# ov2slam/ov2slam

Hardware: AMD Instinct MI355X
Metric: frames/sec tracking + local-BA iters/sec, EuRoC MH_01 stereo 'accurate', 1 GPU vs CPU ref (higher is better)
Workload: dtype u8/int32 fixed point + f32 (LK), f64 (BA)

## Files before the change

### ov2slam_amd/csrc/clahe.hip

```cpp
#include "common.hpp"
#include "xcd_map.hpp"
#include <math.h>
#include <mutex>
#include <type_traits>

#pragma clang fp contract(off)

__device__ __forceinline__ int c_reflect101(int p, int len)
{
    if (len == 1) return 0;
    while (p < 0 || p >= len) p = p < 0 ? -p : 2 * len - 2 - p;
    return p;
}

struct ClaheParams {
    int w, h, stride, tiles_x, tiles_y, tw, th, clip;
    float lut_scale, inv_tw, inv_th;
    long long src_item_stride, dst_item_stride;
    int dst_stride;
    int border;
    int batch, gx_lut;
    int ysplit;
    int nstrips, nlut;
    long long l1_delta;
// ... 165 lines not shown
    __shared__ __attribute__((aligned(16))) uint32_t hist_all[4][CH_MULTI_DW];
    const int wave = __builtin_amdgcn_readfirstlane(threadIdx.x >> 6), lane = threadIdx.x & 63;
    const int ntiles = P.tiles_x * P.tiles_y;
    int b, bx;
    ov2_xcd_map(blockIdx.x, P.gx_lut, P.batch, &b, &bx);
    uint8_t *lb = lut + (long long)b * ntiles * 256 + 4 * lane;
    clahe_lut_tiles<SRC_ALIGNED>(P, src + (long long)b * P.src_item_stride, hist_all[wave], lane, bx * 4 + wave, ntiles, 4 * P.gx_lut,
                                 [&](int t, uint32_t packed) { *(uint32_t *)(lb + (long long)t * 256) = packed; }, CH_NCOPY);
}

#define CLAHE_MAX_CELLS 48
#define CA_UNROLL 6
typedef float c_f32x2 __attribute__((ext_vector_type(2)));

__device__ __forceinline__ float c_ub(uint32_t q, int k) { return (float)((q >> (8 * k)) & 0xFFu); }

template <bool SRC_ALIGNED>
__global__ __launch_bounds__(512) void k_clahe_apply(ClaheParams P, const uint8_t *__restrict__ src, const uint8_t *__restrict__ lut,
                                                     uint8_t *__restrict__ dst)
{
    extern __shared__ __align__(16) unsigned char clahe_smem[];
    const int ncx = P.tiles_x + 1;
    uint32_t *lut4 = (uint32_t *)clahe_smem;
    int cy, b;
    ov2_xcd_map(blockIdx.x, (P.tiles_y + 1) * P.ysplit, P.batch, &b, &cy);
    const int part = cy % P.ysplit;
    cy /= P.ysplit;
    const int tid = threadIdx.x, nthr = blockDim.x;
    const int ty1 = max(cy - 1, 0), ty2 = min(cy, P.tiles_y - 1);
    const uint8_t *L = lut + (long long)b * P.tiles_x * P.tiles_y * 256;
    for (int e = tid; e < ncx * 64; e += nthr) {
        const int cx = e >> 6, v4 = (e & 63) * 4;
        const int tx1 = max(cx - 1, 0), tx2 = min(cx, P.tiles_x - 1);
        const uint32_t a = *(const uint32_t *)(L + (ty1 * P.tiles_x + tx1) * 256 + v4), bb = *(const uint32_t *)(L + (ty1 * P.tiles_x + tx2) * 256 + v4);
        const uint32_t c = *(const uint32_t *)(L + (ty2 * P.tiles_x + tx1) * 256 + v4), d = *(const uint32_t *)(L + (ty2 * P.tiles_x + tx2) * 256 + v4);
        const uint32_t ab01 = __builtin_amdgcn_perm(bb, a, 0x05010400u), ab23 = __builtin_amdgcn_perm(bb, a, 0x07030602u);
        const uint32_t cd01 = __builtin_amdgcn_perm(d, c, 0x05010400u), cd23 = __builtin_amdgcn_perm(d, c, 0x07030602u);
        c_u32x4 o;
        o.x = __builtin_amdgcn_perm(cd01, ab01, 0x05040100u); o.y = __builtin_amdgcn_perm(cd01, ab01, 0x07060302u);
        o.z = __builtin_amdgcn_perm(cd23, ab23, 0x05040100u); o.w = __builtin_amdgcn_perm(cd23, ab23, 0x07060302u);
        *(c_u32x4 *)(lut4 + (cx << 8) + v4) = o;
    }
    __syncthreads();
    int y0 = max(0, (int)floorf(((float)cy - 0.5f) * (float)P.th) - 1), y1 = min(P.h, (int)ceilf(((float)cy + 0.5f) * (float)P.th) + 2);
    while (y0 < y1 && (int)floorf((float)y0 * P.inv_th - 0.5f) + 1 != cy) y0++;
    while (y1 > y0 && (int)floorf((float)(y1 - 1) * P.inv_th - 0.5f) + 1 != cy) y1--;
    if (P.ysplit > 1) {
        const int chunk = (y1 - y0 + P.ysplit - 1) / P.ysplit;
        y0 = min(y1, y0 + part * chunk);
        y1 = min(y1, y0 + chunk);
    }
    const uint8_t *simg = src + (long long)b * P.src_item_stride;
    uint8_t *dimg = dst + (long long)b * P.dst_item_stride;
    const bool dst_aligned = ((P.dst_stride | (int)(size_t)dimg) & 3) == 0;
    constexpr bool src_aligned = SRC_ALIGNED;
    const uint8_t *simg_end = simg + (long long)(P.h - 1) * P.stride + P.w;
    const int ndw = (P.w + 3) >> 2;
    for (int dwi = tid; dwi < ndw; dwi += nthr) {
        const int xb = 4 * dwi;
        float xa[4], xa1[4];
        const uint32_t *lutc[4];
#pragma unroll
        for (int k = 0; k < 4; k++) {
            const int x = min(xb + k, P.w - 1);
            const float txf = (float)x * P.inv_tw - 0.5f;
            const int fx = (int)floorf(txf);
            xa[k] = txf - (float)fx; xa1[k] = 1.0f - xa[k];
            lutc[k] = lut4 + ((fx + 1) << 8);
        }
        const c_f32x2 XA01 = {xa[0], xa[1]}, XA23 = {xa[2], xa[3]}, XB01 = {xa1[0], xa1[1]}, XB23 = {xa1[2], xa1[3]};
        const bool full = dst_aligned && xb + 3 < P.w;
        auto load_rows = [&](int yb, uint32_t (&inr)[CA_UNROLL]) {
#pragma unroll
            for (int u = 0; u < CA_UNROLL; u++) {
                const int y = min(yb + u, y1 - 1);
                const uint8_t *sp = simg + (long long)y * P.stride + xb;
                uint32_t in = 0;
                if (src_aligned) in = *(const uint32_t *)sp;
                else {
                    const uint32_t ph = (uint32_t)((size_t)sp & 3);
                    const uint8_t *ap = sp - ph;
                    if (xb + 3 < P.w && ap + 8 <= simg_end) {
                        const uint32_t lo = *(const uint32_t *)ap, hi = *(const uint32_t *)(ap + 4);
                        in = __builtin_amdgcn_alignbyte(hi, lo, ph);
                    } else for (int k = 0; k < 4; k++) if (xb + k < P.w) in |= (uint32_t)sp[k] << (8 * k);
                }
                inr[u] = in;
            }
        };
        uint32_t inr[CA_UNROLL], nxt[CA_UNROLL];
        if (y0 < y1) load_rows(y0, inr);
        for (int yb = y0; yb < y1; yb += CA_UNROLL) {
            load_rows(yb + CA_UNROLL, nxt);
#pragma unroll
            for (int u = 0; u < CA_UNROLL; u++) {
                const int y = yb + u;
                if (y >= y1) break;
                const float tyf = (float)y * P.inv_th - 0.5f;
                const float ya = tyf - (float)(cy - 1), ya1 = 1.0f - ya;
                const c_f32x2 YA = {ya, ya}, YB = {ya1, ya1};
                uint8_t *drow = dimg + y * P.dst_stride;
                const uint32_t in = inr[u];
                const uint32_t q0 = lutc[0][in & 0xFF], q1 = lutc[1][(in >> 8) & 0xFF], q2 = lutc[2][(in >> 16) & 0xFF], q3 = lutc[3][in >> 24];
                const c_f32x2 A11 = {c_ub(q0, 0), c_ub(q1, 0)}, A12 = {c_ub(q0, 1), c_ub(q1, 1)}, A21 = {c_ub(q0, 2), c_ub(q1, 2)}, A22 = {c_ub(q0, 3), c_ub(q1, 3)};
                const c_f32x2 B11 = {c_ub(q2, 0), c_ub(q3, 0)}, B12 = {c_ub(q2, 1), c_ub(q3, 1)}, B21 = {c_ub(q2, 2), c_ub(q3, 2)}, B22 = {c_ub(q2, 3), c_ub(q3, 3)};
                const c_f32x2 r01 = (A11 * XB01 + A12 * XA01) * YB + (A21 * XB01 + A22 * XA01) * YA;
                const c_f32x2 r23 = (B11 * XB23 + B12 * XA23) * YB + (B21 * XB23 + B22 * XA23) * YA;
                uint32_t out = __builtin_amdgcn_cvt_pk_u8_f32(rintf(r01.x), 0, 0u);
                out = __builtin_amdgcn_cvt_pk_u8_f32(rintf(r01.y), 1, out);
                out = __builtin_amdgcn_cvt_pk_u8_f32(rintf(r23.x), 2, out);
                out = __builtin_amdgcn_cvt_pk_u8_f32(rintf(r23.y), 3, out);
                if (full) *(uint32_t *)(drow + xb) = out;
                else for (int k = 0; k < 4; k++) if (xb + k < P.w) drow[xb + k] = (uint8_t)(out >> (8 * k));
            }
#pragma unroll
            for (int u = 0; u < CA_UNROLL; u++) inr[u] = nxt[u];
        }
    }
    if (P.border > 0) {
        __threadfence_block();
        __syncthreads();
        const int win = P.border, pbl = (win + 3) & ~3, wend = (P.w + win + 3) & ~3, rbeg = P.w & ~3;
        const int ndw_lr = pbl / 4 + ((wend - rbeg) >> 2), ndw_row = (pbl + wend) >> 2;
        auto put = [&](int yt, int ysrc, int c0) {
            const uint8_t *srow = dimg + ysrc * P.dst_stride;
            uint32_t v;
            if (c0 >= 0 && c0 + 3 < P.w) v = *(const uint32_t *)(srow + c0);
            else {
                v = 0;
#pragma unroll
                for (int k = 0; k < 4; k++) {
                    int c = c0 + k;
                    c = c < -win ? -win : (c > P.w + win - 1 ? P.w + win - 1 : c);
                    v |= (uint32_t)srow[c_reflect101(c, P.w)] << (8 * k);
                }
            }
            *(uint32_t *)(dimg + yt * P.dst_stride + c0) = v;
        };
        for (int row = tid >> 3; row < y1 - y0; row += nthr >> 3)
            for (int d = tid & 7; d < ndw_lr; d += 8)
                put(y0 + row, y0 + row, d < pbl / 4 ? 4 * d - pbl : rbeg + 4 * (d - pbl / 4));
        for (int k = max(1, y0); k <= min(win, y1 - 1); k++)
            for (int d = tid; d < ndw_row; d += nthr) put(-k, k, 4 * d - pbl);
        for (int k = max(1, P.h - y1); k <= min(win, P.h - 1 - y0); k++)
            for (int d = tid; d < ndw_row; d += nthr) put(P.h - 1 + k, P.h - 1 - k, 4 * d - pbl);
    }
}

__device__ __forceinline__ uint32_t c_wave_shr1(uint32_t v) { return (uint32_t)__builtin_amdgcn_update_dpp(0, (int)v, 0x138, 0xF, 0xF, true); }
__device__ __forceinline__ uint32_t c_wave_shl1(uint32_t v) { return (uint32_t)__builtin_amdgcn_update_dpp(0, (int)v, 0x130, 0xF, 0xF, true); }

#define CS_UNROLL 6
#define CS_MAX_STRIPS 8
#define CS_LUT_PRIO 3
template <bool UNAL, bool FUSED>
__global__ __launch_bounds__(64 * (CS_MAX_STRIPS + 2), 6) void k_clahe_apply_pyr(ClaheParams P, const uint8_t *__restrict__ src, const uint8_t *__restrict__ lut,
                                                                                uint8_t *__restrict__ dst)
{
    extern __shared__ __align__(16) unsigned char clahe_smem[];
    uint32_t *lut4 = (uint32_t *)clahe_smem;
    uint8_t *ring = clahe_smem + (size_t)(P.tiles_x + 1) * 1024;
    const int b = blockIdx.x, s = __builtin_amdgcn_readfirstlane(threadIdx.x >> 6);
    const int lane = threadIdx.x & 63, ndw = (P.w + 3) >> 2, wr = UNAL ? (P.w & 3) : 0;
    uint32_t *hist_w = (uint32_t *)(ring + (size_t)2 * P.tiles_x * 256) + (s < P.nstrips ? s * CH_WAVE_DW : P.nstrips * CH_WAVE_DW + (s - P.nstrips) * CH_MULTI_DW);
    const int hist_copies = s < P.nstrips ? 1 : CH_NCOPY;
    auto lut_row = [&](int ty, int tx0, int txstep) {
        uint8_t *slot = ring + (size_t)(ty & 1) * P.tiles_x * 256 - (size_t)ty * P.tiles_x * 256 + 4 * lane;
        clahe_lut_tiles<!UNAL>(P, src + (long long)b * P.src_item_stride, hist_w, lane, ty * P.tiles_x + tx0, (ty + 1) * P.tiles_x, txstep,
                               [&](int t, uint32_t packed) { *(uint32_t *)(slot + (size_t)t * 256) = packed; }, hist_copies);
    };
    typedef uint32_t cs_u32_a1 __attribute__((aligned(1)));
    const int cmin = 0, ncell = P.tiles_x + 1;
    const uint8_t *L = lut + (long long)b * P.tiles_x * P.tiles_y * 256;
    auto cell_row = [&](int y) { return (int)floorf((float)y * P.inv_th - 0.5f) + 1; };
    int cy = -1, y_switch = 0;
    auto build = [&](int cyv) {
        const int ty1 = max(cyv - 1, 0), ty2 = min(cyv, P.tiles_y - 1);
        const uint8_t *L1 = FUSED ? ring + (size_t)(ty1 & 1) * P.tiles_x * 256 : L + (size_t)ty1 * P.tiles_x * 256;
        const uint8_t *L2 = FUSED ? ring + (size_t)(ty2 & 1) * P.tiles_x * 256 : L + (size_t)ty2 * P.tiles_x * 256;
        __syncthreads();
        for (int e = threadIdx.x; e < ncell * 64; e += blockDim.x) {
            const int cx = cmin + (e >> 6), v4 = (e & 63) * 4;
            const int tx1 = max(cx - 1, 0), tx2 = min(cx, P.tiles_x - 1);
            const uint32_t a = *(const uint32_t *)(L1 + tx1 * 256 + v4), bb = *(const uint32_t *)(L1 + tx2 * 256 + v4);
            const uint32_t c = *(const uint32_t *)(L2 + tx1 * 256 + v4), dd = *(const uint32_t *)(L2 + tx2 * 256 + v4);
            const uint32_t ab01 = __builtin_amdgcn_perm(bb, a, 0x05010400u), ab23 = __builtin_amdgcn_perm(bb, a, 0x07030602u);
            const uint32_t cd01 = __builtin_amdgcn_perm(dd, c, 0x05010400u), cd23 = __builtin_amdgcn_perm(dd, c, 0x07030602u);
            c_u32x4 o;
            o.x = __builtin_amdgcn_perm(cd01, ab01, 0x05040100u); o.y = __builtin_amdgcn_perm(cd01, ab01, 0x07060302u);
            o.z = __builtin_amdgcn_perm(cd23, ab23, 0x05040100u); o.w = __builtin_amdgcn_perm(cd23, ab23, 0x07060302u);
            *(c_u32x4 *)(lut4 + ((e >> 6) << 8) + v4) = o;
        }
        __syncthreads();
    };
    if (FUSED) {
        lut_row(0, s, P.nstrips + P.nlut);
        if (s >= P.nstrips) {
            const int n_cell_rows = cell_row(P.h - 1) + 1;
            __builtin_amdgcn_s_setprio(CS_LUT_PRIO);
            for (int c = 0; c < n_cell_rows; c++) {
                build(c);
                if (c + 1 < P.tiles_y) lut_row(c + 1, s - P.nstrips, P.nlut);
            }
            return;
        }
    }
    const int core0 = s == 0 ? 0 : 63 + 62 * (s - 1);
    const int core1 = s == P.nstrips - 1 ? ndw : 63 + 62 * s;
    const int d_first = s == 0 ? 0 : core0 - 1;
    const int d_raw = d_first + lane;
    const int d = min(d_raw, ndw - 1);
    const bool core = d_raw >= core0 && d_raw < core1;
    const int xb = 4 * d;
    float xa[4], xa1[4];
    const uint32_t *lutc[4];
#pragma unroll
    for (int k = 0; k < 4; k++) {
        const float txf = (float)min(xb + k, P.w - 1) * P.inv_tw - 0.5f;
        const int fx = (int)floorf(txf);
        xa[k] = txf - (float)fx; xa1[k] = 1.0f - xa[k];
        lutc[k] = lut4 + ((fx + 1 - cmin) << 8);
    }
    const c_f32x2 XA01 = {xa[0], xa[1]}, XA23 = {xa[2], xa[3]}, XB01 = {xa1[0], xa1[1]}, XB23 = {xa1[2], xa1[3]};
    uint8_t *dimg = dst + (long long)b * P.dst_item_stride;
    uint8_t *l1 = dimg + P.l1_delta;
    const int win = P.border;
    const int l1odd = UNAL ? (P.l1_w & 1) : 0;
    const int nb0 = (win + 3) >> 2, nb1 = (win + 1) >> 1;
    const int nbr0 = nb0 + (wr ? 1 : 0), nbr1 = nb1 + l1odd;
    const bool bl0 = core && d < nb0, br0 = core && d >= ndw - nbr0;
    const bool bl1 = core && d >= 1 && d <= nb1, br1 = core && d >= ndw - nbr1;
    const bool edge_strip = s == 0 || core1 > ndw - max(nbr0, nbr1);
    const bool first_col = d_raw == 0, last_col = d_raw == ndw - 1;
    const bool dup = d_raw > ndw - 1;
    const uint32_t pad0 = 4u * nb0, pad1 = 2u * nb1;
    const uint32_t slack0 = pad0 + 4u * (uint32_t)((P.w + win + 3) >> 2), slack1 = pad1 + 2u * (uint32_t)((P.l1_w + win + 3) >> 1);
    const uint32_t o0 = dup ? slack0 : pad0 + 4u * d;
    const uint32_t o0b = bl0 ? pad0 - 4u * (d + 1) : (br0 ? pad0 + (uint32_t)(2 * P.w - 2 - xb - ((wr & 1) ? 0 : 2)) : slack0);
    const uint32_t sel_br = (wr & 1) ? 0x01020304u : 0x03040506u;
    const uint32_t sel_fix = (last_col && wr) ? (wr == 1 ? 0x01020304u : (wr == 2 ? 0x03040504u : 0x05060504u)) : 0x07060504u;
    const uint32_t sel_rt = wr == 0 ? 0x0c0c0c06u : (wr == 1 ? 0x0c0c0c00u : (wr == 2 ? 0x0c0c0c02u : 0x0c0c0c04u));
    const uint32_t o1 = core ? pad1 + 2u * d : slack1;
    const uint32_t o1b = bl1 ? pad1 - 2u * d : (br1 ? pad1 + (uint32_t)P.l1_w + 2u * (ndw - 1 - d) - (uint32_t)l1odd : slack1);
    const bool fix1 = last_col && l1odd;
    uint8_t *d0m = dimg - pad0, *d1m = l1 - pad1;
    const uint32_t xo = (d == ndw - 1 && wr) ? (uint32_t)(P.w - 4) : (uint32_t)xb;
    const uint32_t in_sh = (d == ndw - 1 && wr) ? 8u * (4u - (uint32_t)wr) : 0u;

    auto stage = [&](int y) {
        cy = cell_row(y);
        int yn = max(y + 1, (int)(((float)cy + 0.5f) * (float)P.th) - 2);
        while (yn < P.h && cell_row(yn) == cy) yn++;
        y_switch = yn;
        build(cy);
    };
    uint8_t *dbase = min(d0m - (long long)win * P.dst_stride, d1m - (long long)win * P.l1_pitch) - 256;
    const __amdgpu_buffer_rsrc_t rs_dst = __builtin_amdgcn_make_buffer_rsrc(dbase, 0, 0x7fffffff, 0x00020000);
    const uint8_t *sbase = src + (long long)b * P.src_item_stride;
    const __amdgpu_buffer_rsrc_t rs_src = __builtin_amdgcn_make_buffer_rsrc((void *)sbase, 0, 0x7fffffff, 0x00020000);
    auto put0 = [&](uint8_t *row, uint32_t v, uint32_t bv) {
        const int so = (int)(row - dbase);
        __builtin_amdgcn_raw_buffer_store_b32(v, rs_dst, (int)o0, so, 0);
        if (edge_strip) __builtin_amdgcn_raw_buffer_store_b32(bv, rs_dst, (int)o0b, so, 0);
    };
    auto put1 = [&](uint8_t *row, uint32_t v, uint32_t bv) {
        const int so = (int)(row - dbase);
        __builtin_amdgcn_raw_buffer_store_b16((unsigned short)v, rs_dst, (int)o1, so, 0);
        if (edge_strip) __builtin_amdgcn_raw_buffer_store_b16((unsigned short)bv, rs_dst, (int)o1b, so, 0);
    };
    typedef unsigned short cu16x2 __attribute__((ext_vector_type(2)));
    uint8_t *r1 = d1m;
    auto emit = [&](int Y, uint32_t c0, uint32_t c1, uint32_t c2, uint32_t c3, uint32_t c4, auto mirror_c) {
        constexpr bool MIRROR = decltype(mirror_c)::value;
        const cu16x2 s0 = __builtin_bit_cast(cu16x2, c0), s1 = __builtin_bit_cast(cu16x2, c1), s2 = __builtin_bit_cast(cu16x2, c2),
                     s3 = __builtin_bit_cast(cu16x2, c3), s4 = __builtin_bit_cast(cu16x2, c4);
        const cu16x2 v = (s2 * (unsigned short)6 + (s1 + s3) * (unsigned short)4 + s0 + s4 + (unsigned short)128) >> (unsigned short)8;
        uint32_t o = __builtin_amdgcn_perm(0u, __builtin_bit_cast(uint32_t, v), 0x0c0c0200u);
        uint32_t bv = 0;
        if (edge_strip) {
            bv = __builtin_amdgcn_perm(c_wave_shr1(o), o, 0x0c0c0500u);
            if (UNAL && fix1) o = bv;
        }
        put1(r1, o, bv);
        r1 += P.l1_pitch;
        if (MIRROR) {
            if (Y >= 1 && Y <= win) put1(d1m - (long long)Y * P.l1_pitch, o, bv);
            if (Y >= P.l1_h - 1 - win && Y <= P.l1_h - 2) put1(d1m + (long long)(2 * (P.l1_h - 1) - Y) * P.l1_pitch, o, bv);
        }
    };

    uint32_t hA = 0, hB = 0, hC = 0, hD = 0, hE = 0;
    const uint8_t *srow = src + (long long)b * P.src_item_stride;
    uint8_t *r0 = d0m;
    uint32_t inr[CS_UNROLL], nxt[CS_UNROLL];
#pragma unroll
    for (int u = 0; u < CS_UNROLL; u++) inr[u] = *(const cs_u32_a1 *)(srow + (long long)min(u, P.h - 1) * P.stride + xo) >> (UNAL ? in_sh : 0u);
    srow += (long long)CS_UNROLL * P.stride;
    auto do_row = [&](int y, uint32_t in, auto mirror_c) {
        constexpr bool MIRROR = decltype(mirror_c)::value;
        const float tyf = (float)y * P.inv_th - 0.5f;
        const float ya = tyf - (float)(cy - 1), ya1 = 1.0f - ya;
        const c_f32x2 YA = {ya, ya}, YB = {ya1, ya1};
        const uint32_t q0 = lutc[0][in & 0xFF], q1 = lutc[1][(in >> 8) & 0xFF], q2 = lutc[2][(in >> 16) & 0xFF], q3 = lutc[3][in >> 24];
        const c_f32x2 A11 = {c_ub(q0, 0), c_ub(q1, 0)}, A12 = {c_ub(q0, 1), c_ub(q1, 1)}, A21 = {c_ub(q0, 2), c_ub(q1, 2)}, A22 = {c_ub(q0, 3), c_ub(q1, 3)};
        const c_f32x2 B11 = {c_ub(q2, 0), c_ub(q3, 0)}, B12 = {c_ub(q2, 1), c_ub(q3, 1)}, B21 = {c_ub(q2, 2), c_ub(q3, 2)}, B22 = {c_ub(q2, 3), c_ub(q3, 3)};
        const c_f32x2 r01 = (A11 * XB01 + A12 * XA01) * YB + (A21 * XB01 + A22 * XA01) * YA;
        const c_f32x2 r23 = (B11 * XB23 + B12 * XA23) * YB + (B21 * XB23 + B22 * XA23) * YA;
        const c_f32x2 MAGIC = {12582912.0f, 12582912.0f};
        const c_f32x2 m01 = r01 + MAGIC, m23 = r23 + MAGIC;
        const uint32_t u0 = __builtin_bit_cast(uint32_t, (float)m01.x), u1 = __builtin_bit_cast(uint32_t, (float)m01.y);
        const uint32_t u2 = __builtin_bit_cast(uint32_t, (float)m23.x), u3 = __builtin_bit_cast(uint32_t, (float)m23.y);
        uint32_t out = __builtin_amdgcn_perm(__builtin_amdgcn_perm(u3, u2, 0x0c0c0400u), __builtin_amdgcn_perm(u1, u0, 0x0c0c0400u), 0x05040100u);
        uint32_t lf = c_wave_shr1(out), rt = c_wave_shl1(out);
        if (first_col) lf = __builtin_amdgcn_perm(out, out, 0x01020000u);
        if (edge_strip) {
            if (UNAL) out = __builtin_amdgcn_perm(out, lf, sel_fix);
        }
        if (UNAL) { if (last_col) rt = __builtin_amdgcn_perm(out, lf, sel_rt); }
        else if (last_col) rt = out >> 16;
        uint32_t bv = 0;
        if (edge_strip)
            bv = bl0 ? __builtin_amdgcn_perm(out, rt, 0x05060700u) : __builtin_amdgcn_perm(out, lf, sel_br);
        put0(r0, out, bv);
        r0 += P.dst_stride;
        if (MIRROR) {
            if (y >= 1 && y <= win) put0(d0m - (long long)y * P.dst_stride, out, bv);
            if (y >= P.h - 1 - win && y <= P.h - 2) put0(d0m + (long long)(2 * (P.h - 1) - y) * P.dst_stride, out, bv);
        }
        const uint32_t l0 = __builtin_amdgcn_alignbyte(out, lf, 2);
        const uint32_t h0 = __builtin_amdgcn_udot4(l0, 0x04060401u, __builtin_amdgcn_udot4(out, 0x00010000u, 0u, false), false);
        const uint32_t h1 = __builtin_amdgcn_udot4(out, 0x04060401u, __builtin_amdgcn_udot4(rt, 0x00000001u, 0u, false), false);
        hA = hB; hB = hC; hC = hD; hD = hE; hE = h0 | (h1 << 16);
    };
    for (int yb = 0; yb < P.h; yb += CS_UNROLL) {
        if (yb + 2 * CS_UNROLL <= P.h) {
#pragma unroll
            for (int u = 0; u < CS_UNROLL; u++) { nxt[u] = (uint32_t)__builtin_amdgcn_raw_buffer_load_b32(rs_src, (int)xo, (int)(srow - sbase), 0) >> (UNAL ? in_sh : 0u); srow += P.stride; }
        } else {
#pragma unroll
            for (int u = 0; u < CS_UNROLL; u++)
                nxt[u] = *(const cs_u32_a1 *)(src + (long long)b * P.src_item_stride + (long long)min(yb + CS_UNROLL + u, P.h - 1) * P.stride + xo) >> (UNAL ? in_sh : 0u);
        }
        if (yb == y_switch) stage(yb);
        const bool fast = yb > 2 * win + 2 && yb + CS_UNROLL - 1 < P.h - 1 - win && yb + CS_UNROLL - 4 < 2 * (P.l1_h - 1 - win) &&
                          y_switch >= yb + CS_UNROLL && yb + CS_UNROLL <= P.h;
        if (fast) {
#pragma unroll
            for (int u = 0; u < CS_UNROLL; u++) {
                do_row(yb + u, inr[u], std::false_type());
                if ((u & 1) == 0) emit((yb + u - 2) >> 1, hA, hB, hC, hD, hE, std::false_type());
            }
        } else {
#pragma nounroll
            for (int u = 0; u < CS_UNROLL; u++) {
                const int y = yb + u;
                if (y >= P.h) break;
                if (y == y_switch) stage(y);
                do_row(y, inr[0], std::true_type());
                if (!(y & 1)) {
                    if (y == 2) emit(0, hE, hD, hC, hD, hE, std::true_type());
                    else if (y > 2) emit((y - 2) >> 1, hA, hB, hC, hD, hE, std::true_type());
                }
#pragma unroll
                for (int k = 0; k + 1 < CS_UNROLL; k++) inr[k] = inr[k + 1];
            }
        }
#pragma unroll
        for (int u = 0; u < CS_UNROLL; u++) inr[u] = nxt[u];
    }
    if (P.h & 1) emit((P.h - 1) >> 1, hC, hD, hE, hD, hC, std::true_type());
    else emit((P.h - 2) >> 1, hB, hC, hD, hE, hD, std::true_type());
}

int ov2_launch_clahe(ov2_ctx *ctx, const uint8_t *src_d, int w, int h, int stride, size_t src_batch_stride, int batch,
                     double clip_limit, int tiles_x, int tiles_y, uint8_t *dst_d, int dst_stride, size_t dst_batch_stride,
                     uint8_t *lut_d, int border, const PyrDesc *pyr, int *level1_done)
{
    if (level1_done) *level1_done = 0;
    OV2_REQUIRE(tiles_x + 1 <= CLAHE_MAX_CELLS && (size_t)(tiles_x + 1) * 1024 <= 160 * 1024, OV2_EUNSUPPORTED,
                "CLAHE: too many tile columns / too wide an image for the LDS tables");
    static std::once_flag attr_once;
    static hipError_t attr_err = hipSuccess;
    std::call_once(attr_once, [] {
        attr_err = hipFuncSetAttribute((const void *)k_clahe_apply<true>, hipFuncAttributeMaxDynamicSharedMemorySize, 160 * 1024);
        if (attr_err == hipSuccess)
            attr_err = hipFuncSetAttribute((const void *)k_clahe_apply<false>, hipFuncAttributeMaxDynamicSharedMemorySize, 160 * 1024);
    });
    OV2_HIP_CHECK(attr_err);
    ClaheParams P;
    P.border = border;
    P.nstrips = 0; P.nlut = 0; P.l1_delta = 0; P.l1_pitch = P.l1_w = P.l1_h = 0;
    int ew = w, eh = h;
    if (!(w % tiles_x == 0 && h % tiles_y == 0)) { ew = w + (tiles_x - w % tiles_x); eh = h + (tiles_y - h % tiles_y); }
    P.w = w; P.h = h; P.stride = stride; P.tiles_x = tiles_x; P.tiles_y = tiles_y;
    P.tw = ew / tiles_x; P.th = eh / tiles_y;
    const int total = P.tw * P.th;
    P.lut_scale = (float)(256 - 1) / (float)total;
    P.clip = 0;
    if (clip_limit > 0.0) { P.clip = (int)(clip_limit * total / 256); if (P.clip < 1) P.clip = 1; }
    P.inv_tw = 1.0f / (float)P.tw; P.inv_th = 1.0f / (float)P.th;
    P.src_item_stride = (long long)src_batch_stride; P.dst_item_stride = (long long)dst_batch_stride; P.dst_stride = dst_stride;
    const int tiles_per_wave = (long long)batch * tiles_x * tiles_y >= 32768 ? 5 : 1;
    const bool src_al = ((stride | (int)(size_t)src_d | (int)src_batch_stride) & 3) == 0;
    P.ysplit = (long long)batch * (tiles_y + 1) >= 256 ? 1 : (P.th >= 48 ? 6 : (P.th >= 16 ? 3 : 1));
    P.batch = batch; P.gx_lut = (tiles_x * tiles_y + 4 * tiles_per_wave - 1) / (4 * tiles_per_wave);
    bool lut_launched = false;
    auto launch_lut = [&] {
        if (!lut_launched) hipLaunchKernelGGL(src_al ? k_clahe_lut<true> : k_clahe_lut<false>, dim3(P.gx_lut * batch), dim3(256), 0, ctx->stream, P, src_d, lut_d);
        lut_launched = true;
    };
    if (pyr && pyr->n_levels >= 2 && border == pyr->win && w >= 64 && h >= 8 && 2 * ((border + 3) / 4) + 1 <= (w + 3) / 4 &&
        (((size_t)dst_d | (size_t)dst_stride | dst_batch_stride) & 3) == 0 && (pyr->lv[1].img_pitch & 1) == 0) {
        const int ndw = (w + 3) / 4, nstrips = ndw <= 64 ? 1 : 2 + (ndw - 126 + 61) / 62;
        const bool want = ctx->clahe_strips >= 0 ? ctx->clahe_strips >= 1 : (long long)batch * nstrips >= 1024;
        if (want && nstrips <= CS_MAX_STRIPS && tiles_x + 1 <= 40) {
            static std::once_flag strip_once;
            static hipError_t strip_err = hipSuccess;
            std::call_once(strip_once, [] {
                const void *fn[4] = {(const void *)k_clahe_apply_pyr<false, false>, (const void *)k_clahe_apply_pyr<true, false>,
                                     (const void *)k_clahe_apply_pyr<false, true>, (const void *)k_clahe_apply_pyr<true, true>};
                for (int i = 0; i < 4 && strip_err == hipSuccess; i++) strip_err = hipFuncSetAttribute(fn[i], hipFuncAttributeMaxDynamicSharedMemorySize, 72 * 1024);
            });
            OV2_HIP_CHECK(strip_err);
            P.nstrips = nstrips;
            P.l1_delta = pyr->lv[1].img_roi - pyr->lv[0].img_roi; P.l1_pitch = pyr->lv[1].img_pitch; P.l1_w = pyr->lv[1].w; P.l1_h = pyr->lv[1].h;
            const bool unal = (w & 3) != 0 || (pyr->lv[1].w & 1) != 0;
            const int nlut = tiles_x <= 16 ? 1 : std::max(1, std::min((tiles_x + 7) / 8, CS_MAX_STRIPS + 2 - nstrips));
            const bool fused = (ctx->clahe_strips == 2 || (ctx->clahe_strips < 0 && tiles_x <= 16 * nlut)) && (unal || src_al);
            if (fused) {
                P.nlut = nlut;
                const size_t lds = (size_t)(tiles_x + 1) * 1024 + (size_t)2 * tiles_x * 256 + ((size_t)nstrips * CH_WAVE_DW + (size_t)P.nlut * CH_MULTI_DW) * 4;
                hipLaunchKernelGGL((unal ? k_clahe_apply_pyr<true, true> : k_clahe_apply_pyr<false, true>), dim3(batch), dim3(64 * (nstrips + P.nlut)), lds, ctx->stream, P, src_d, lut_d, dst_d);
            } else {
                launch_lut();
                hipLaunchKernelGGL((unal ? k_clahe_apply_pyr<true, false> : k_clahe_apply_pyr<false, false>), dim3(batch), dim3(64 * nstrips), (size_t)(tiles_x + 1) * 1024, ctx->stream, P, src_d, lut_d, dst_d);
            }
            OV2_HIP_CHECK(hipGetLastError());
            if (level1_done) *level1_done = 1;
            return OV2_OK;
        }
    }
    launch_lut();
    const size_t apply_lds = (size_t)(tiles_x + 1) * 1024;
    const int ndw = (w + 3) / 4, passes = (ndw + 511) / 512;
    const int apply_threads = (((ndw + passes - 1) / passes) + 63) / 64 * 64;
    hipLaunchKernelGGL(src_al ? k_clahe_apply<true> : k_clahe_apply<false>, dim3((tiles_y + 1) * P.ysplit * batch), dim3(apply_threads), apply_lds, ctx->stream, P, src_d, lut_d, dst_d);
    OV2_HIP_CHECK(hipGetLastError());
    return OV2_OK;
}

extern "C" {

int ov2_clahe_d(ov2_ctx *ctx, const uint8_t *src_d, int w, int h, int stride, size_t src_batch_stride, int batch,
                double clip_limit, int tiles_x, int tiles_y, uint8_t *dst_d, int dst_stride, size_t dst_batch_stride)
{
    OV2_REQUIRE(ctx && src_d && dst_d, OV2_EINVAL, "NULL argument");
    OV2_REQUIRE(w > 0 && h > 0 && stride >= w && dst_stride >= w && batch >= 1 && tiles_x > 0 && tiles_y > 0, OV2_EINVAL, "bad geometry");
    OV2_REQUIRE(tiles_x <= w && tiles_y <= h, OV2_EINVAL, "more tiles than pixels");
    OV2_HIP_CHECK(hipSetDevice(ctx->device));
    const size_t lut_bytes = (size_t)batch * tiles_x * tiles_y * 256;
    const int rc = ctx->reserve_device(lut_bytes);
    if (rc != OV2_OK) return rc;
    return ov2_launch_clahe(ctx, src_d, w, h, stride, src_batch_stride, batch, clip_limit, tiles_x, tiles_y, dst_d, dst_stride,
                            dst_batch_stride, (uint8_t *)ctx->d_scratch, 0, nullptr, nullptr);
}

int ov2_pyr_build_clahe_d(ov2_ctx *ctx, ov2_pyr *p, const uint8_t *img_d, int stride, size_t img_batch_stride,
                          double clip_limit, int tiles_x, int tiles_y)
{
    OV2_REQUIRE(ctx && p && img_d, OV2_EINVAL, "NULL argument");
    OV2_REQUIRE(stride >= p->w && tiles_x > 0 && tiles_y > 0 && tiles_x <= p->w && tiles_y <= p->h, OV2_EINVAL, "bad geometry");
    OV2_REQUIRE(p->d.batch == 1 || img_batch_stride >= (size_t)stride * (size_t)p->h, OV2_EINVAL, "img_batch_stride too small");
    OV2_HIP_CHECK(hipSetDevice(ctx->device));
    const size_t lut_bytes = (size_t)p->d.batch * tiles_x * tiles_y * 256;
    int rc = ctx->reserve_device(lut_bytes);
    if (rc != OV2_OK) return rc;
    const PyrLevelDesc &L0 = p->d.lv[0];
    int l1_done = 0;
    rc = ov2_launch_clahe(ctx, img_d, p->w, p->h, stride, img_batch_stride, p->d.batch, clip_limit, tiles_x, tiles_y,
                          p->d.base + L0.img_roi, L0.img_pitch, (size_t)p->d.item_stride, (uint8_t *)ctx->d_scratch, p->d.win,
                          &p->d, &l1_done);
    if (rc != OV2_OK) return rc;
    rc = ov2_launch_pyr_build(ctx, p, nullptr, 0, 0, l1_done);
    if (rc != OV2_OK) return rc;
    return ov2_pyr_mark_ready(ctx, p);
}

int ov2_pyr_build_clahe_h(ov2_ctx *ctx, ov2_pyr *p, const uint8_t *img_h, int stride, double clip_limit, int tiles_x, int tiles_y)
{
    OV2_REQUIRE(ctx && p && img_h, OV2_EINVAL, "NULL argument");
    OV2_REQUIRE(p->d.batch == 1, OV2_EINVAL, "host-buffer entry point takes batch=1 pyramids");
    OV2_REQUIRE(stride >= p->w && tiles_x > 0 && tiles_y > 0 && tiles_x <= p->w && tiles_y <= p->h, OV2_EINVAL, "bad geometry");
    OV2_HIP_CHECK(hipSetDevice(ctx->device));
    const size_t pitch = ((size_t)p->w + 15) & ~(size_t)15;
    const size_t img = (pitch * p->h + 255) & ~(size_t)255, lut_bytes = (size_t)tiles_x * tiles_y * 256;
    int rc = ctx->reserve_device(img + lut_bytes);
    if (rc != OV2_OK) return rc;
    uint8_t *ds = (uint8_t *)ctx->d_scratch;
    rc = ctx->upload_image(ds, pitch, img_h, (size_t)stride, (size_t)p->w, (size_t)p->h);
    if (rc != OV2_OK) return rc;
    const PyrLevelDesc &L0 = p->d.lv[0];
    int l1_done = 0;
    rc = ov2_launch_clahe(ctx, ds, p->w, p->h, (int)pitch, 0, 1, clip_limit, tiles_x, tiles_y, p->d.base + L0.img_roi, L0.img_pitch,
                          (size_t)p->d.item_stride, ds + img, p->d.win, &p->d, &l1_done);
    if (rc != OV2_OK) return rc;
    rc = ov2_launch_pyr_build(ctx, p, nullptr, 0, 0, l1_done);
    if (rc != OV2_OK) return rc;
    return ov2_pyr_mark_ready(ctx, p);
}

int ov2_pyr_build_clahe_hb(ov2_ctx *ctx, ov2_pyr *p, int n_items, const uint8_t *const *img_h, int stride, double clip_limit, int tiles_x, int tiles_y)
{
    OV2_REQUIRE(ctx && p && img_h, OV2_EINVAL, "NULL argument");
    OV2_REQUIRE(p->parent == nullptr, OV2_EINVAL, "an item view is read-only");
    OV2_REQUIRE(n_items >= 1 && n_items <= p->d.batch, OV2_EINVAL, "n_items out of range");
    const bool use_clahe = clip_limit >= 0.0;
    OV2_REQUIRE(stride >= p->w && (!use_clahe || (tiles_x > 0 && tiles_y > 0 && tiles_x <= p->w && tiles_y <= p->h)), OV2_EINVAL, "bad geometry");
    for (int b = 0; b < n_items; b++) OV2_REQUIRE(img_h[b] != nullptr, OV2_EINVAL, "NULL image");
    OV2_HIP_CHECK(hipSetDevice(ctx->device));
    const size_t pitch = ((size_t)p->w + 15) & ~(size_t)15;
    const size_t img = (pitch * p->h + 255) & ~(size_t)255, lut_bytes = use_clahe ? (size_t)n_items * tiles_x * tiles_y * 256 : 0;
    int rc = ctx->reserve_device(img * (size_t)n_items + lut_bytes);
    if (rc != OV2_OK) return rc;
    uint8_t *ds = (uint8_t *)ctx->d_scratch;
// ... 40 lines not shown
```

Measured before the change: 1.190 million.

## Specialize CLAHE apply loop on edge strips and prefetch LUT gathers ahead

Wraps the row walk of the fused CLAHE+pyramid kernel in a template lambda specialized on whether the wave handles an edge strip, so interior strips drop the per-row edge branches and extra stores. The LDS LUT gathers are split from the blend math and issued several rows ahead (all rows when fused, three otherwise) to hide LDS latency. All source loads now go through buffer loads, offsets are kept as 32-bit ints, and the fused variant's occupancy hint drops from 6 to 5 to allow more registers. The cost is larger code and higher register pressure, which may reduce occupancy.

```diff
diff --git a/ov2slam_amd/csrc/clahe.hip b/ov2slam_amd/csrc/clahe.hip
--- a/ov2slam_amd/csrc/clahe.hip
+++ b/ov2slam_amd/csrc/clahe.hip
@@ -341,9 +341,10 @@
 
 #define CS_UNROLL 6
 #define CS_MAX_STRIPS 8
+#define CS_AHEAD_PLAIN 3
 #define CS_LUT_PRIO 3
 template <bool UNAL, bool FUSED>
-__global__ __launch_bounds__(64 * (CS_MAX_STRIPS + 2), 6) void k_clahe_apply_pyr(ClaheParams P, const uint8_t *__restrict__ src, const uint8_t *__restrict__ lut,
+__global__ __launch_bounds__(64 * (CS_MAX_STRIPS + 2), FUSED ? 5 : 6) void k_clahe_apply_pyr(ClaheParams P, const uint8_t *__restrict__ src, const uint8_t *__restrict__ lut,
                                                                                 uint8_t *__restrict__ dst)
 {
     extern __shared__ __align__(16) unsigned char clahe_smem[];
@@ -358,7 +359,6 @@
         clahe_lut_tiles<!UNAL>(P, src + (long long)b * P.src_item_stride, hist_w, lane, ty * P.tiles_x + tx0, (ty + 1) * P.tiles_x, txstep,
                                [&](int t, uint32_t packed) { *(uint32_t *)(slot + (size_t)t * 256) = packed; }, hist_copies);
     };
-    typedef uint32_t cs_u32_a1 __attribute__((aligned(1)));
     const int cmin = 0, ncell = P.tiles_x + 1;
     const uint8_t *L = lut + (long long)b * P.tiles_x * P.tiles_y * 256;
     auto cell_row = [&](int y) { return (int)floorf((float)y * P.inv_th - 0.5f) + 1; };
@@ -428,6 +428,8 @@
     const uint32_t o0b = bl0 ? pad0 - 4u * (d + 1) : (br0 ? pad0 + (uint32_t)(2 * P.w - 2 - xb - ((wr & 1) ? 0 : 2)) : slack0);
     const uint32_t sel_br = (wr & 1) ? 0x01020304u : 0x03040506u;
     const uint32_t sel_fix = (last_col && wr) ? (wr == 1 ? 0x01020304u : (wr == 2 ? 0x03040504u : 0x05060504u)) : 0x07060504u;
+    const uint32_t sel_lf = first_col ? 0x05060404u : 0x03020100u;
+    const uint32_t sel_rt0 = last_col ? 0x0c0c0706u : 0x03020100u;
     const uint32_t sel_rt = wr == 0 ? 0x0c0c0c06u : (wr == 1 ? 0x0c0c0c00u : (wr == 2 ? 0x0c0c0c02u : 0x0c0c0c04u));
     const uint32_t o1 = core ? pad1 + 2u * d : slack1;
     const uint32_t o1b = bl1 ? pad1 - 2u * d : (br1 ? pad1 + (uint32_t)P.l1_w + 2u * (ndw - 1 - d) - (uint32_t)l1odd : slack1);
@@ -447,118 +449,127 @@
     const __amdgpu_buffer_rsrc_t rs_dst = __builtin_amdgcn_make_buffer_rsrc(dbase, 0, 0x7fffffff, 0x00020000);
     const uint8_t *sbase = src + (long long)b * P.src_item_stride;
     const __amdgpu_buffer_rsrc_t rs_src = __builtin_amdgcn_make_buffer_rsrc((void *)sbase, 0, 0x7fffffff, 0x00020000);
-    auto put0 = [&](uint8_t *row, uint32_t v, uint32_t bv) {
-        const int so = (int)(row - dbase);
-        __builtin_amdgcn_raw_buffer_store_b32(v, rs_dst, (int)o0, so, 0);
-        if (edge_strip) __builtin_amdgcn_raw_buffer_store_b32(bv, rs_dst, (int)o0b, so, 0);
+    const int d0o = (int)(d0m - dbase), d1o = (int)(d1m - dbase);
+    auto load_row = [&](int so) { return (uint32_t)__builtin_amdgcn_raw_buffer_load_b32(rs_src, (int)xo, so, 0) >> (UNAL ? in_sh : 0u); };
+    typedef unsigned short cu16x2 __attribute__((ext_vector_type(2)));
+
+    auto walk = [&](auto edge_c) {
+        constexpr bool EDGE = decltype(edge_c)::value;
+        auto put0 = [&](int so, uint32_t v, uint32_t bv) {
+            __builtin_amdgcn_raw_buffer_store_b32(v, rs_dst, (int)o0, so, 0);
+            if (EDGE) __builtin_amdgcn_raw_buffer_store_b32(bv, rs_dst, (int)o0b, so, 0);
+        };
+        auto put1 = [&](int so, uint32_t v, uint32_t bv) {
+            __builtin_amdgcn_raw_buffer_store_b16((unsigned short)v, rs_dst, (int)o1, so, 0);
+            if (EDGE) __builtin_amdgcn_raw_buffer_store_b16((unsigned short)bv, rs_dst, (int)o1b, so, 0);
+        };
+        int r1 = d1o;
+        auto emit = [&](int Y, uint32_t c0, uint32_t c1, uint32_t c2, uint32_t c3, uint32_t c4, auto mirror_c) {
+            constexpr bool MIRROR = decltype(mirror_c)::value;
+            const cu16x2 s0 = __builtin_bit_cast(cu16x2, c0), s1 = __builtin_bit_cast(cu16x2, c1), s2 = __builtin_bit_cast(cu16x2, c2),
+                         s3 = __builtin_bit_cast(cu16x2, c3), s4 = __builtin_bit_cast(cu16x2, c4);
+            const cu16x2 v = (s2 * (unsigned short)6 + (s1 + s3) * (unsigned short)4 + s0 + s4 + (unsigned short)128) >> (unsigned short)8;
+            uint32_t o = __builtin_amdgcn_perm(0u, __builtin_bit_cast(uint32_t, v), 0x0c0c0200u);
+            uint32_t bv = 0;
+            if (EDGE) {
+                bv = __builtin_amdgcn_perm(c_wave_shr1(o), o, 0x0c0c0500u);
+                if (UNAL && fix1) o = bv;
+            }
+            put1(r1, o, bv);
+            r1 += P.l1_pitch;
+            if (MIRROR) {
+                if (Y >= 1 && Y <= win) put1(d1o - Y * P.l1_pitch, o, bv);
+                if (Y >= P.l1_h - 1 - win && Y <= P.l1_h - 2) put1(d1o + (2 * (P.l1_h - 1) - Y) * P.l1_pitch, o, bv);
+            }
+        };
+
+        uint32_t hA = 0, hB = 0, hC = 0, hD = 0, hE = 0;
+        int srow = CS_UNROLL * P.stride;
+        int r0 = d0o;
+        uint32_t inr[CS_UNROLL], nxt[CS_UNROLL];
+#pragma unroll
+        for (int u = 0; u < CS_UNROLL; u++) inr[u] = load_row(min(u, P.h - 1) * P.stride);
+        struct RowIn { uint32_t q0, q1, q2, q3; };
+        auto gather = [&](uint32_t in) { return RowIn{lutc[0][in & 0xFF], lutc[1][(in >> 8) & 0xFF], lutc[2][(in >> 16) & 0xFF], lutc[3][in >> 24]}; };
+        auto blend = [&](int y, const RowIn &g, auto mirror_c) {
+            constexpr bool MIRROR = decltype(mirror_c)::value;
+            const uint32_t q0 = g.q0, q1 = g.q1, q2 = g.q2, q3 = g.q3;
+            const float tyf = (float)y * P.inv_th - 0.5f;
+            const float ya = tyf - (float)(cy - 1), ya1 = 1.0f - ya;
+            const c_f32x2 YA = {ya, ya}, YB = {ya1, ya1};
+            const c_f32x2 A11 = {c_ub(q0, 0), c_ub(q1, 0)}, A12 = {c_ub(q0, 1), c_ub(q1, 1)}, A21 = {c_ub(q0, 2), c_ub(q1, 2)}, A22 = {c_ub(q0, 3), c_ub(q1, 3)};
+            const c_f32x2 B11 = {c_ub(q2, 0), c_ub(q3, 0)}, B12 = {c_ub(q2, 1), c_ub(q3, 1)}, B21 = {c_ub(q2, 2), c_ub(q3, 2)}, B22 = {c_ub(q2, 3), c_ub(q3, 3)};
+            const c_f32x2 r01 = (A11 * XB01 + A12 * XA01) * YB + (A21 * XB01 + A22 * XA01) * YA;
+            const c_f32x2 r23 = (B11 * XB23 + B12 * XA23) * YB + (B21 * XB23 + B22 * XA23) * YA;
+            const c_f32x2 MAGIC = {12582912.0f, 12582912.0f};
+            const c_f32x2 m01 = r01 + MAGIC, m23 = r23 + MAGIC;
+            const uint32_t u0 = __builtin_bit_cast(uint32_t, (float)m01.x), u1 = __builtin_bit_cast(uint32_t, (float)m01.y);
+            const uint32_t u2 = __builtin_bit_cast(uint32_t, (float)m23.x), u3 = __builtin_bit_cast(uint32_t, (float)m23.y);
+            uint32_t out = __builtin_amdgcn_perm(__builtin_amdgcn_perm(u3, u2, 0x0c0c0400u), __builtin_amdgcn_perm(u1, u0, 0x0c0c0400u), 0x05040100u);
+            uint32_t lf = c_wave_shr1(out), rt = c_wave_shl1(out);
+            uint32_t bv = 0;
+            if (EDGE) {
+                lf = __builtin_amdgcn_perm(out, lf, sel_lf);
+                if (UNAL) out = __builtin_amdgcn_perm(out, lf, sel_fix);
+                if (UNAL) { if (last_col) rt = __builtin_amdgcn_perm(out, lf, sel_rt); }
+                else rt = __builtin_amdgcn_perm(out, rt, sel_rt0);
+                bv = bl0 ? __builtin_amdgcn_perm(out, rt, 0x05060700u) : __builtin_amdgcn_perm(out, lf, sel_br);
+            }
+            put0(r0, out, bv);
+            r0 += P.dst_stride;
+            if (MIRROR) {
+                if (y >= 1 && y <= win) put0(d0o - y * P.dst_stride, out, bv);
+                if (y >= P.h - 1 - win && y <= P.h - 2) put0(d0o + (2 * (P.h - 1) - y) * P.dst_stride, out, bv);
+            }
+            const uint32_t l0 = __builtin_amdgcn_alignbyte(out, lf, 2);
+            const uint32_t h0 = __builtin_amdgcn_udot4(l0, 0x04060401u, __builtin_amdgcn_udot4(out, 0x00010000u, 0u, false), false);
+            const uint32_t h1 = __builtin_amdgcn_udot4(out, 0x04060401u, __builtin_amdgcn_udot4(rt, 0x00000001u, 0u, false), false);
+            hA = hB; hB = hC; hC = hD; hD = hE; hE = h0 | (h1 << 16);
+        };
+        for (int yb = 0; yb < P.h; yb += CS_UNROLL) {
+            if (yb + 2 * CS_UNROLL <= P.h) {
+#pragma unroll
+                for (int u = 0; u < CS_UNROLL; u++) { nxt[u] = load_row(srow); srow += P.stride; }
+            } else {
+#pragma unroll
+                for (int u = 0; u < CS_UNROLL; u++) nxt[u] = load_row(min(yb + CS_UNROLL + u, P.h - 1) * P.stride);
+            }
+            if (yb == y_switch) stage(yb);
+            const bool fast = yb > 2 * win + 2 && yb + CS_UNROLL - 1 < P.h - 1 - win && yb + CS_UNROLL - 4 < 2 * (P.l1_h - 1 - win) &&
+                              y_switch >= yb + CS_UNROLL && yb + CS_UNROLL <= P.h;
+            if (fast) {
+                constexpr int AHEAD = FUSED ? CS_UNROLL : CS_AHEAD_PLAIN;
+                RowIn g[CS_UNROLL];
+#pragma unroll
+                for (int u = 0; u < AHEAD; u++) g[u] = gather(inr[u]);
+#pragma unroll
+                for (int u = 0; u < CS_UNROLL; u++) {
+                    blend(yb + u, g[u], std::false_type());
+                    if (u + AHEAD < CS_UNROLL) g[u + AHEAD] = gather(inr[u + AHEAD]);
+                    if ((u & 1) == 0) emit((yb + u - 2) >> 1, hA, hB, hC, hD, hE, std::false_type());
+                }
+            } else {
+#pragma nounroll
+                for (int u = 0; u < CS_UNROLL; u++) {
+                    const int y = yb + u;
+                    if (y >= P.h) break;
+                    if (y == y_switch) stage(y);
+                    blend(y, gather(inr[0]), std::true_type());
+                    if (!(y & 1)) {
+                        if (y == 2) emit(0, hE, hD, hC, hD, hE, std::true_type());
+                        else if (y > 2) emit((y - 2) >> 1, hA, hB, hC, hD, hE, std::true_type());
+                    }
+#pragma unroll
+                    for (int k = 0; k + 1 < CS_UNROLL; k++) inr[k] = inr[k + 1];
+                }
+            }
+#pragma unroll
+            for (int u = 0; u < CS_UNROLL; u++) inr[u] = nxt[u];
+        }
+        if (P.h & 1) emit((P.h - 1) >> 1, hC, hD, hE, hD, hC, std::true_type());
+        else emit((P.h - 2) >> 1, hB, hC, hD, hE, hD, std::true_type());
     };
-    auto put1 = [&](uint8_t *row, uint32_t v, uint32_t bv) {
-        const int so = (int)(row - dbase);
-        __builtin_amdgcn_raw_buffer_store_b16((unsigned short)v, rs_dst, (int)o1, so, 0);
-        if (edge_strip) __builtin_amdgcn_raw_buffer_store_b16((unsigned short)bv, rs_dst, (int)o1b, so, 0);
-    };
-    typedef unsigned short cu16x2 __attribute__((ext_vector_type(2)));
-    uint8_t *r1 = d1m;
-    auto emit = [&](int Y, uint32_t c0, uint32_t c1, uint32_t c2, uint32_t c3, uint32_t c4, auto mirror_c) {
-        constexpr bool MIRROR = decltype(mirror_c)::value;
-        const cu16x2 s0 = __builtin_bit_cast(cu16x2, c0), s1 = __builtin_bit_cast(cu16x2, c1), s2 = __builtin_bit_cast(cu16x2, c2),
-                     s3 = __builtin_bit_cast(cu16x2, c3), s4 = __builtin_bit_cast(cu16x2, c4);
-        const cu16x2 v = (s2 * (unsigned short)6 + (s1 + s3) * (unsigned short)4 + s0 + s4 + (unsigned short)128) >> (unsigned short)8;
-        uint32_t o = __builtin_amdgcn_perm(0u, __builtin_bit_cast(uint32_t, v), 0x0c0c0200u);
-        uint32_t bv = 0;
-        if (edge_strip) {
-            bv = __builtin_amdgcn_perm(c_wave_shr1(o), o, 0x0c0c0500u);
-            if (UNAL && fix1) o = bv;
-        }
-        put1(r1, o, bv);
-        r1 += P.l1_pitch;
-        if (MIRROR) {
-            if (Y >= 1 && Y <= win) put1(d1m - (long long)Y * P.l1_pitch, o, bv);
-            if (Y >= P.l1_h - 1 - win && Y <= P.l1_h - 2) put1(d1m + (long long)(2 * (P.l1_h - 1) - Y) * P.l1_pitch, o, bv);
-        }
-    };
-
-    uint32_t hA = 0, hB = 0, hC = 0, hD = 0, hE = 0;
-    const uint8_t *srow = src + (long long)b * P.src_item_stride;
-    uint8_t *r0 = d0m;
-    uint32_t inr[CS_UNROLL], nxt[CS_UNROLL];
-#pragma unroll
-    for (int u = 0; u < CS_UNROLL; u++) inr[u] = *(const cs_u32_a1 *)(srow + (long long)min(u, P.h - 1) * P.stride + xo) >> (UNAL ? in_sh : 0u);
-    srow += (long long)CS_UNROLL * P.stride;
-    auto do_row = [&](int y, uint32_t in, auto mirror_c) {
-        constexpr bool MIRROR = decltype(mirror_c)::value;
-        const float tyf = (float)y * P.inv_th - 0.5f;
-        const float ya = tyf - (float)(cy - 1), ya1 = 1.0f - ya;
-        const c_f32x2 YA = {ya, ya}, YB = {ya1, ya1};
-        const uint32_t q0 = lutc[0][in & 0xFF], q1 = lutc[1][(in >> 8) & 0xFF], q2 = lutc[2][(in >> 16) & 0xFF], q3 = lutc[3][in >> 24];
-        const c_f32x2 A11 = {c_ub(q0, 0), c_ub(q1, 0)}, A12 = {c_ub(q0, 1), c_ub(q1, 1)}, A21 = {c_ub(q0, 2), c_ub(q1, 2)}, A22 = {c_ub(q0, 3), c_ub(q1, 3)};
-        const c_f32x2 B11 = {c_ub(q2, 0), c_ub(q3, 0)}, B12 = {c_ub(q2, 1), c_ub(q3, 1)}, B21 = {c_ub(q2, 2), c_ub(q3, 2)}, B22 = {c_ub(q2, 3), c_ub(q3, 3)};
-        const c_f32x2 r01 = (A11 * XB01 + A12 * XA01) * YB + (A21 * XB01 + A22 * XA01) * YA;
-        const c_f32x2 r23 = (B11 * XB23 + B12 * XA23) * YB + (B21 * XB23 + B22 * XA23) * YA;
-        const c_f32x2 MAGIC = {12582912.0f, 12582912.0f};
-        const c_f32x2 m01 = r01 + MAGIC, m23 = r23 + MAGIC;
-        const uint32_t u0 = __builtin_bit_cast(uint32_t, (float)m01.x), u1 = __builtin_bit_cast(uint32_t, (float)m01.y);
-        const uint32_t u2 = __builtin_bit_cast(uint32_t, (float)m23.x), u3 = __builtin_bit_cast(uint32_t, (float)m23.y);
-        uint32_t out = __builtin_amdgcn_perm(__builtin_amdgcn_perm(u3, u2, 0x0c0c0400u), __builtin_amdgcn_perm(u1, u0, 0x0c0c0400u), 0x05040100u);
-        uint32_t lf = c_wave_shr1(out), rt = c_wave_shl1(out);
-        if (first_col) lf = __builtin_amdgcn_perm(out, out, 0x01020000u);
-        if (edge_strip) {
-            if (UNAL) out = __builtin_amdgcn_perm(out, lf, sel_fix);
-        }
-        if (UNAL) { if (last_col) rt = __builtin_amdgcn_perm(out, lf, sel_rt); }
-        else if (last_col) rt = out >> 16;
-        uint32_t bv = 0;
-        if (edge_strip)
-            bv = bl0 ? __builtin_amdgcn_perm(out, rt, 0x05060700u) : __builtin_amdgcn_perm(out, lf, sel_br);
-        put0(r0, out, bv);
-        r0 += P.dst_stride;
-        if (MIRROR) {
-            if (y >= 1 && y <= win) put0(d0m - (long long)y * P.dst_stride, out, bv);
-            if (y >= P.h - 1 - win && y <= P.h - 2) put0(d0m + (long long)(2 * (P.h - 1) - y) * P.dst_stride, out, bv);
-        }
-        const uint32_t l0 = __builtin_amdgcn_alignbyte(out, lf, 2);
-        const uint32_t h0 = __builtin_amdgcn_udot4(l0, 0x04060401u, __builtin_amdgcn_udot4(out, 0x00010000u, 0u, false), false);
-        const uint32_t h1 = __builtin_amdgcn_udot4(out, 0x04060401u, __builtin_amdgcn_udot4(rt, 0x00000001u, 0u, false), false);
-        hA = hB; hB = hC; hC = hD; hD = hE; hE = h0 | (h1 << 16);
-    };
-    for (int yb = 0; yb < P.h; yb += CS_UNROLL) {
-        if (yb + 2 * CS_UNROLL <= P.h) {
-#pragma unroll
-            for (int u = 0; u < CS_UNROLL; u++) { nxt[u] = (uint32_t)__builtin_amdgcn_raw_buffer_load_b32(rs_src, (int)xo, (int)(srow - sbase), 0) >> (UNAL ? in_sh : 0u); srow += P.stride; }
-        } else {
-#pragma unroll
-            for (int u = 0; u < CS_UNROLL; u++)
-                nxt[u] = *(const cs_u32_a1 *)(src + (long long)b * P.src_item_stride + (long long)min(yb + CS_UNROLL + u, P.h - 1) * P.stride + xo) >> (UNAL ? in_sh : 0u);
-        }
-        if (yb == y_switch) stage(yb);
-        const bool fast = yb > 2 * win + 2 && yb + CS_UNROLL - 1 < P.h - 1 - win && yb + CS_UNROLL - 4 < 2 * (P.l1_h - 1 - win) &&
-                          y_switch >= yb + CS_UNROLL && yb + CS_UNROLL <= P.h;
-        if (fast) {
-#pragma unroll
-            for (int u = 0; u < CS_UNROLL; u++) {
-                do_row(yb + u, inr[u], std::false_type());
-                if ((u & 1) == 0) emit((yb + u - 2) >> 1, hA, hB, hC, hD, hE, std::false_type());
-            }
-        } else {
-#pragma nounroll
-            for (int u = 0; u < CS_UNROLL; u++) {
-                const int y = yb + u;
-                if (y >= P.h) break;
-                if (y == y_switch) stage(y);
-                do_row(y, inr[0], std::true_type());
-                if (!(y & 1)) {
-                    if (y == 2) emit(0, hE, hD, hC, hD, hE, std::true_type());
-                    else if (y > 2) emit((y - 2) >> 1, hA, hB, hC, hD, hE, std::true_type());
-                }
-#pragma unroll
-                for (int k = 0; k + 1 < CS_UNROLL; k++) inr[k] = inr[k + 1];
-            }
-        }
-#pragma unroll
-        for (int u = 0; u < CS_UNROLL; u++) inr[u] = nxt[u];
-    }
-    if (P.h & 1) emit((P.h - 1) >> 1, hC, hD, hE, hD, hC, std::true_type());
-    else emit((P.h - 2) >> 1, hB, hC, hD, hE, hD, std::true_type());
+    if (edge_strip) walk(std::true_type()); else walk(std::false_type());
 }
 
 int ov2_launch_clahe(ov2_ctx *ctx, const uint8_t *src_d, int w, int h, int stride, size_t src_batch_stride, int batch,
```

Result: no change. 1.197 million (median of 6 runs) (+0.6%).
